# hammershock/3dgs-avatar-release

Measured on AMD Instinct MI355X. Metric: render fps (fwd+bwd) @200k Gaussians 1024x1024 SH3, higher is better.
Workload: dtype f32; 1 GPU; config3: 200k Gaussians, 1024x1024, SH deg 3, forward+backward; shs+scales+rotations inputs, L1 loss (L1 fused into the rasterizer: l1_target); tile_rect=1, l1=fused, long_lists=0, gaussians=200000, width=1024, height=1024, sh_degree=3, frames_per_rank=1857, total_frames=1857, ranks=1, backend=none, parallelism=frames sharded x1

## Files before the change

### 3dgs-avatar-release_amd/csrc/render_bwd.hip

```cpp
#include "common.h"
#include "blend.h"

__device__ __forceinline__ float ring_ror1(float v) {
    return __builtin_bit_cast(float, __builtin_amdgcn_update_dpp(0, __builtin_bit_cast(int, v), 0x121, 0xF, 0xF, true));
}
#define RING 16
#define RING_STRIDE 48

typedef float bwd_f4 __attribute__((ext_vector_type(4)));
template <bool SECOND>
__device__ __forceinline__ void split_accumulate(float (&x)[9], float (&y)[9], unsigned long long mask, float Gd, float dx,
                                                 float dy, float tdx, float tdy, float wgt, float gx, float gy,
                                                 float gz, unsigned long long m1, uint32_t lds_addr, bwd_f4& q0, bwd_f4& q1,
                                                 bwd_f4& q2, float& rot0, float& rot1) {
    unsigned long long save;
    asm volatile(
        "s_mov_b64 %[sv], exec\n\t"
        "s_mov_b64 exec, %[m]\n\t"
        "v_fmac_f32 %[x0], %[Gd], %[dx]\n\t"
        "v_fmac_f32 %[x1], %[Gd], %[dy]\n\t"
        "v_fmac_f32 %[x2], %[tdx], %[dx]\n\t"
        "v_fmac_f32 %[x3], %[tdx], %[dy]\n\t"
        "v_fmac_f32 %[x4], %[tdy], %[dy]\n\t"
        "v_add_f32 %[x5], %[x5], %[Gd]\n\t"
        "v_fmac_f32 %[x6], %[w], %[gx]\n\t"
        "v_fmac_f32 %[x7], %[w], %[gy]\n\t"
        "v_fmac_f32 %[x8], %[w], %[gz]\n\t"
        "s_mov_b64 exec, %[sv]"
        : [x0] "+v"(x[0]), [x1] "+v"(x[1]), [x2] "+v"(x[2]), [x3] "+v"(x[3]), [x4] "+v"(x[4]), [x5] "+v"(x[5]), [x6] "+v"(x[6]),
          [x7] "+v"(x[7]), [x8] "+v"(x[8]), [sv] "=&s"(save)
        : [m] "s"(mask), [Gd] "v"(Gd), [dx] "v"(dx), [dy] "v"(dy), [tdx] "v"(tdx), [tdy] "v"(tdy), [w] "v"(wgt), [gx] "v"(gx),
          [gy] "v"(gy), [gz] "v"(gz)
        : "scc");
#define GS_ACC_Y                                     \
        "s_andn2_b64 exec, %[sv], %[m]\n\t"          \
        "v_fmac_f32 %[y0], %[Gd], %[dx]\n\t"         \
        "v_fmac_f32 %[y1], %[Gd], %[dy]\n\t"         \
        "v_fmac_f32 %[y2], %[tdx], %[dx]\n\t"        \
        "v_fmac_f32 %[y3], %[tdx], %[dy]\n\t"        \
        "v_fmac_f32 %[y4], %[tdy], %[dy]\n\t"        \
        "v_add_f32 %[y5], %[y5], %[Gd]\n\t"          \
        "v_fmac_f32 %[y6], %[w], %[gx]\n\t"          \
        "v_fmac_f32 %[y7], %[w], %[gy]\n\t"          \
        "v_fmac_f32 %[y8], %[w], %[gz]\n\t"          \
        "s_mov_b64 exec, %[sv]\n\t"                  \
        "v_mov_b32_dpp %[r0], %[r0] row_ror:1 row_mask:0xf bank_mask:0xf bound_ctrl:1\n\t" \
        "v_mov_b32_dpp %[r1], %[r1] row_ror:1 row_mask:0xf bank_mask:0xf bound_ctrl:1\n\t" \
        "s_waitcnt lgkmcnt(0)"
#define GS_ACC_Y_OUT [y0] "+v"(y[0]), [y1] "+v"(y[1]), [y2] "+v"(y[2]), [y3] "+v"(y[3]), [y4] "+v"(y[4]), [y5] "+v"(y[5]), \
                     [y6] "+v"(y[6]), [y7] "+v"(y[7]), [y8] "+v"(y[8]), [q0] "+v"(q0), [q1] "+v"(q1), [r0] "+v"(rot0), [r1] "+v"(rot1), \
                     [sv] "=&s"(save)
#define GS_ACC_Y_IN [m] "s"(mask), [m1] "s"(m1), [a] "v"(lds_addr), [Gd] "v"(Gd), [dx] "v"(dx), [dy] "v"(dy), [tdx] "v"(tdx), \
                    [tdy] "v"(tdy), [w] "v"(wgt), [gx] "v"(gx), [gy] "v"(gy), [gz] "v"(gz)
    if constexpr (SECOND) {
        asm volatile(
            "s_mov_b64 %[sv], exec\n\t"
            "s_andn2_b64 exec, %[m1], %[m]\n\t"
            "ds_read_b128 %[q0], %[a]\n\t"
            "ds_read_b128 %[q1], %[a] offset:16\n\t"
            "ds_read_b128 %[q2], %[a] offset:32\n\t" GS_ACC_Y
            : GS_ACC_Y_OUT, [q2] "+v"(q2)
            : GS_ACC_Y_IN
            : "memory", "scc");
    } else {
        asm volatile(
            "s_mov_b64 %[sv], exec\n\t"
            "s_andn2_b64 exec, %[m1], %[m]\n\t"
            "ds_read_b128 %[q0], %[a]\n\t"
            "ds_read_b128 %[q1], %[a] offset:16\n\t"
            "ds_read_b32 %[q2], %[a] offset:32\n\t" GS_ACC_Y
            : GS_ACC_Y_OUT, [q2] "+v"(q2.x)
            : GS_ACC_Y_IN
            : "memory", "scc");
    }
#undef GS_ACC_Y
#undef GS_ACC_Y_OUT
#undef GS_ACC_Y_IN
}

struct EntryQ {
    bwd_f4 q0, q1, q2;
};
#define ENT_SLOTS 2

template <bool SECOND>
__device__ __forceinline__ void switch_entry(EntryQ& e, uint32_t lds_addr, unsigned long long m0, unsigned long long m1) {
    unsigned long long save;
    if constexpr (SECOND) {
        asm volatile(
            "s_mov_b64 %[sv], exec\n\t"
            "s_andn2_b64 exec, %[m1], %[m0]\n\t"
            "ds_read_b128 %[q0], %[a]\n\t"
            "ds_read_b128 %[q1], %[a] offset:16\n\t"
            "ds_read_b128 %[q2], %[a] offset:32\n\t"
            "s_mov_b64 exec, %[sv]\n\t"
            "s_waitcnt lgkmcnt(0)"
            : [q0] "+v"(e.q0), [q1] "+v"(e.q1), [q2] "+v"(e.q2), [sv] "=&s"(save)
            : [a] "v"(lds_addr), [m0] "s"(m0), [m1] "s"(m1)
            : "memory", "scc");
    } else {
        float b = e.q2.x;
        asm volatile(
            "s_mov_b64 %[sv], exec\n\t"
            "s_andn2_b64 exec, %[m1], %[m0]\n\t"
            "ds_read_b128 %[q0], %[a]\n\t"
            "ds_read_b128 %[q1], %[a] offset:16\n\t"
            "ds_read_b32 %[b], %[a] offset:32\n\t"
            "s_mov_b64 exec, %[sv]\n\t"
            "s_waitcnt lgkmcnt(0)"
            : [q0] "+v"(e.q0), [q1] "+v"(e.q1), [b] "+v"(b), [sv] "=&s"(save)
            : [a] "v"(lds_addr), [m0] "s"(m0), [m1] "s"(m1)
            : "memory", "scc");
        e.q2.x = b;
    }
}

#ifndef BWD_MIN_WAVES
#define BWD_MIN_WAVES 1
#endif
#ifndef BWD_MAX_WAVES
#define BWD_MAX_WAVES (BWD_MIN_WAVES > 6 ? BWD_MIN_WAVES : 6)
#endif
template <int MODE>
__attribute__((amdgpu_waves_per_eu(BWD_MIN_WAVES, BWD_MAX_WAVES)))
__global__ __launch_bounds__(64, BWD_MIN_WAVES) void render_bwd_kernel(const float4* __restrict__ rec,
                                                        const uint2* __restrict__ ranges,
                                                        const uint32_t* __restrict__ order, int W, int H, int gx,
                                                        int ntiles, int xmap,
                                                        const uint32_t* __restrict__ qlist,
                                                        const uint32_t* __restrict__ ncon_c,
                                                        const uint32_t* __restrict__ qcount,
                                                        const float* __restrict__ out_color,
                                                        const float* __restrict__ dL_dpix,
                                                        const float* __restrict__ dL_dopa,
                                                        const float* __restrict__ final_T, const float* __restrict__ bg,
                                                        float4* __restrict__ qrows, uint32_t* __restrict__ q8,
                                                        const float4* __restrict__ ckpt,
                                                        const uint32_t* __restrict__ ck_start, const int chunks,
                                                        const int blocks_per_chunk, const SecondImage second,
                                                        const L1Grad l1, const float l1_inv_n) {
    constexpr bool OPA = MODE == 1, SECOND = MODE == 2, SONES = MODE == 3;
    if constexpr (SECOND) { if (*second.all_ones != 0u) return; }
    if constexpr (SONES) { if (*second.all_ones == 0u) return; }
    constexpr int NP2 = SECOND ? 5 : 3;
    __shared__ float2 pix[NP2][4 * RING_STRIDE];
    __shared__ bwd_f4 ent[ENT_SLOTS][RING][3];
    int slot, q;
    const int chunk = chunks > 1 ? (int)blockIdx.x / blocks_per_chunk : 0;
    render_block_map((int)blockIdx.x - chunk * blocks_per_chunk, xmap, &slot, &q);
    if (slot >= ntiles) return;
    const int tile = (int)(order[slot] & 0x7FFFFFFFu);
    const int tx = tile % gx, ty = tile / gx;
    const int lane = threadIdx.x;
    const int j = lane & (RING - 1), ring = lane / RING;
    const int QX0 = tx * TILE + 8 * (q & 1), QY0 = ty * TILE + 8 * (q >> 1);
    const int pi = (RING - j) & (RING - 1), pl = ring * RING + pi;
    const int px = QX0 + (pl & 7), py = QY0 + (pl >> 3);
    const uint2 range = ranges[tile];
    const int n = (int)(range.y - range.x);
    const int m_all = (int)qcount[tile * 4 + q];
    const uint32_t ks = chunk > 0 ? ck_start[(size_t)(tile * 4 + q) * (size_t)chunks + chunk] : 0u;
    if (ks >= (uint32_t)m_all) return;
    const int k0 = (int)ks;
    const uint32_t ke = chunk + 1 < chunks ? ck_start[(size_t)(tile * 4 + q) * (size_t)chunks + chunk + 1] : 0xFFFFFFFFu;
    const int m = (int)min(ke, (uint32_t)m_all) - k0;
    if (m <= 0) return;
    const uint32_t qbase = 4u * range.x + (uint32_t)q * (uint32_t)n + (uint32_t)k0;
    const float4 zero4 = make_float4(0.f, 0.f, 0.f, 0.f);
    float gtot0, T0 = 1.0f;
    {
        float4 c0 = zero4, c1 = make_float4((float)px, (float)py, __uint_as_float((uint32_t)pi), 0.f);
        float3 h = make_float3(0.f, 0.f, 0.f);
        if (px < W && py < H) {
            const size_t HW = (size_t)H * W;
            const size_t pid = (size_t)py * W + px;
            float g0 = 0.f, g1 = 0.f, g2 = 0.f;
            if (dL_dpix) { g0 = dL_dpix[pid]; g1 = dL_dpix[HW + pid]; g2 = dL_dpix[2 * HW + pid]; }
            const float o0 = out_color[pid], o1 = out_color[HW + pid], o2 = out_color[2 * HW + pid];
            if (l1.target) {
                const float sc = (l1.grad ? l1.grad[0] : 1.0f) * l1_inv_n;
                const float d0 = o0 - l1.target[pid], d1 = o1 - l1.target[HW + pid], d2 = o2 - l1.target[2 * HW + pid];
                g0 += d0 > 0.f ? sc : (d0 < 0.f ? -sc : 0.f);
                g1 += d1 > 0.f ? sc : (d1 < 0.f ? -sc : 0.f);
                g2 += d2 > 0.f ? sc : (d2 < 0.f ? -sc : 0.f);
            }
            c0 = make_float4(g0, g1, g2, o0 * g0 + o1 * g1 + o2 * g2);
            const uint32_t nc = ncon_c[pid];
            c1.z = __uint_as_float((nc > (uint32_t)k0 ? nc - (uint32_t)k0 : 0u) + (uint32_t)pi);
            if (OPA) {
                const float Tf = final_T[pid];
                c0.w -= dL_dopa[pid] * (Tf * (1.0f - bg[0]));
            }
            if (SECOND || SONES) {
                h = make_float3(second.dL_dpix[pid], second.dL_dpix[HW + pid], second.dL_dpix[2 * HW + pid]);
                if (SECOND) c0.w += second.out_color[pid] * h.x + second.out_color[HW + pid] * h.y + second.out_color[2 * HW + pid] * h.z;
                else c0.w -= (1.0f - second.out_color[pid]) * h.x + (1.0f - second.out_color[HW + pid]) * h.y + (1.0f - second.out_color[2 * HW + pid]) * h.z;
            }
            if (chunk > 0) {
                const size_t ci = ((size_t)(tile * 4 + q) * (size_t)(chunks - 1) + (size_t)(chunk - 1)) * 64 + pl;
                const float4 ck = ckpt[ci];
                T0 = ck.x;
                c0.w -= ck.y * g0 + ck.z * g1 + ck.w * g2;
                if (SECOND) {
                    const float4 ck2 = second.ckpt[ci];
                    c0.w -= ck2.y * h.x + ck2.z * h.y + ck2.w * h.z;
                }
            }
        }
        const int slot = ring * RING_STRIDE + pi;
        pix[0][slot] = pix[0][slot + RING] = make_float2(c0.x, c0.y);
        pix[1][slot] = pix[1][slot + RING] = make_float2(c0.z, c1.x);
        pix[2][slot] = pix[2][slot + RING] = make_float2(c1.y, c1.z);
        if (SECOND) {
            pix[3][slot] = pix[3][slot + RING] = make_float2(h.x, h.y);
            pix[4][slot] = pix[4][slot + RING] = make_float2(h.z, 0.f);
        }
        gtot0 = c0.w;
    }

    float3 q2 = make_float3(0.f, 0.f, 0.f);
    auto stage = [&](const float4 p0, const float4 p1, const float4 p2, const int chunk, uint32_t& row) {
        const uint32_t off = __float_as_uint(p2.y), rmin = __float_as_uint(p2.z), rsz = __float_as_uint(p2.w);
        const uint32_t minx = rmin & 0xFFFFu, miny = rmin >> 16, w = rsz & 0xFFFFu;
        row = gradient_row(off, w, (uint32_t)tx - minx, (uint32_t)ty - miny, (uint32_t)q);
        if (ring == 0) {
            bwd_f4* e = ent[chunk & (ENT_SLOTS - 1)][j];
            e[0] = bwd_f4{p0.x, p0.y, (-0.5f * LOG2E_F) * p0.z, -LOG2E_F * p0.w};
            e[1] = bwd_f4{(-0.5f * LOG2E_F) * p1.x, p1.y, p1.z, p1.w};
            e[2] = bwd_f4{p2.x, q2.x, q2.y, q2.z};
        }
    };
    uint32_t id_ahead = 0;
    auto gather_id = [&](int k) { id_ahead = qlist[qbase + min(k, m - 1)]; };
    auto gather = [&](float4& p0, float4& p1, float4& p2) {
        const uint32_t id = id_ahead;
        p0 = rec[(size_t)id * 3];
        p1 = rec[(size_t)id * 3 + 1];
        p2 = rec[(size_t)id * 3 + 2];
        if (SECOND) q2 = make_float3(second.colors[(size_t)id * 3], second.colors[(size_t)id * 3 + 1], second.colors[(size_t)id * 3 + 2]);
    };

    float4 p0 = zero4, p1 = zero4, p2 = zero4;
    EntryQ cur;
    cur.q0 = cur.q1 = cur.q2 = bwd_f4{0.f, 0.f, 0.f, 0.f};
    uint32_t row_staged = 0;
    gather_id(j);
    gather(p0, p1, p2);
    gather_id(RING + j);
    stage(p0, p1, p2, 0, row_staged);
    gather(p0, p1, p2);
    gather_id(2 * RING + j);
    __syncthreads();
    const uint32_t ent_addr0 = (uint32_t)(uintptr_t)&ent[0][j][0], ent_addr1 = (uint32_t)(uintptr_t)&ent[1][j][0];

    float accA[9], accB[9];
#pragma unroll
    for (int c9 = 0; c9 < 9; c9++) accA[c9] = accB[c9] = 0.f;
    uint32_t rowA = 0, rowB = 0;
    uint32_t pidx = (uint32_t)(ring * RING_STRIDE + pi);
    float2 pc[NP2];
#pragma unroll
    for (int c6 = 0; c6 < NP2; c6++) pc[c6] = pix[c6][pidx];
    float T = T0, Rem = gtot0;

    auto fold_rings = [&](float (&a)[9], float (&f)[3]) {
        float t;
        asm volatile(
            "s_nop 1\n\t"
            "v_permlane16_swap_b32 %[a0], %[a1]\n\t"
            "v_permlane16_swap_b32 %[a2], %[a3]\n\t"
            "v_permlane16_swap_b32 %[a4], %[a5]\n\t"
            "v_permlane16_swap_b32 %[a6], %[a7]\n\t"
            "v_mov_b32 %[t], %[a8]\n\t"
            "v_add_f32 %[a0], %[a0], %[a1]\n\t"
            "v_add_f32 %[a2], %[a2], %[a3]\n\t"
            "v_add_f32 %[a4], %[a4], %[a5]\n\t"
            "v_add_f32 %[a6], %[a6], %[a7]\n\t"
            "v_permlane16_swap_b32 %[a8], %[t]\n\t"
            "v_permlane32_swap_b32 %[a0], %[a2]\n\t"
            "v_permlane32_swap_b32 %[a4], %[a6]\n\t"
            "v_add_f32 %[a8], %[a8], %[t]\n\t"
            "v_add_f32 %[a0], %[a0], %[a2]\n\t"
            "v_add_f32 %[a4], %[a4], %[a6]\n\t"
            "v_mov_b32 %[t], %[a8]\n\t"
            "s_nop 1\n\t"
            "v_permlane32_swap_b32 %[a8], %[t]\n\t"
            "v_add_f32 %[a8], %[a8], %[t]"
            : [a0] "+v"(a[0]), [a1] "+v"(a[1]), [a2] "+v"(a[2]), [a3] "+v"(a[3]), [a4] "+v"(a[4]), [a5] "+v"(a[5]),
              [a6] "+v"(a[6]), [a7] "+v"(a[7]), [a8] "+v"(a[8]), [t] "=&v"(t));
        f[0] = a[0];
        f[1] = a[4];
        f[2] = a[8];
    };
    float* const qrow_words = reinterpret_cast<float*>(qrows);
    auto write_row = [&](size_t row, const float (&f)[3]) {
        qrow_words[row * 8 + ring] = f[0];
        qrow_words[row * 8 + ring + 4] = f[1];
        if (ring == 0) q8[row] = __float_as_uint(f[2]);
    };

    const int total = m + RING - 1;
    auto run_round = [&](const int s0, float (&X)[9], uint32_t& rowX, float (&Y)[9]) {
        const uint32_t row_done = rowX;
        rowX = row_staged;
        const uint32_t ea = (s0 & RING) ? ent_addr1 : ent_addr0;
        switch_entry<SECOND>(cur, ea, 0ull, 0x0001000100010001ull);
        stage(p0, p1, p2, s0 / RING + 1, row_staged);
        gather(p0, p1, p2);
        gather_id(s0 + 3 * RING + j);
        if (s0 >= 2 * RING) {
            float f[3];
            fold_rings(X, f);
            write_row(row_done, f);
        }
        if (s0 > 0) pidx -= (uint32_t)RING;
#pragma unroll
        for (int c9 = 0; c9 < 9; c9++) X[c9] = 0.f;
        const int tend = min(RING, total - s0);
        unsigned long long mx = 0x0001000100010001ull;
        auto step = [&](const int t) {
            const uint32_t s = (uint32_t)(s0 + t);
            const float3 g = make_float3(pc[0].x, pc[0].y, pc[1].x);
            const float pxf = pc[1].y, pyf = pc[2].x;
            const uint32_t lim = __float_as_uint(pc[2].y);
            const float h0 = SECOND ? pc[3].x : 0.f, h1 = SECOND ? pc[3].y : 0.f, h2 = SECOND ? pc[NP2 - 1].x : 0.f;
            pidx += 1u;
#pragma unroll
            for (int c6 = 0; c6 < NP2; c6++) pc[c6] = pix[c6][pidx];
            const float dx = cur.q0.x - pxf, dy = cur.q0.y - pyf;
            const float power2 = __builtin_fmaf(cur.q0.z * dx, dx, __builtin_fmaf(cur.q0.w, dx, cur.q1.x * dy) * dy);
            const float G = __builtin_amdgcn_exp2f(power2);
            const float al = fminf(0.99f, cur.q1.y * G);
            const bool valid = (power2 <= 0.0f) && (s < lim) && (al >= (1.0f / 255.0f));
            const float alpha = valid ? al : 0.f;
            const float Gv = valid ? G : 0.f;
            const float wgt = alpha * T;
            float cg = cur.q1.z * g.x + cur.q1.w * g.y + cur.q2.x * g.z;
            if constexpr (SECOND) cg += cur.q2.y * h0 + cur.q2.z * h1 + cur.q2.w * h2;
            Rem = __builtin_fmaf(-cg, wgt, Rem);
            const float one_m = 1.f - alpha;
            const float dL_dalpha = T * cg - Rem * __builtin_amdgcn_rcpf(one_m);
            T *= one_m;
            const float Gd = Gv * dL_dalpha;
            const float tdx = Gd * dx, tdy = Gd * dy;
            const unsigned long long mx1 = (mx << 1) | 0x0001000100010001ull;
            split_accumulate<SECOND>(X, Y, mx, Gd, dx, dy, tdx, tdy, wgt, g.x, g.y, g.z, mx1, ea, cur.q0, cur.q1, cur.q2, T, Rem);
            mx = mx1;
        };
        int t = 0;
        for (; t + 1 < tend; t += 2) {
            step(t);
            step(t + 1);
        }
        if (t < tend) step(t);
    };
    for (int s0 = 0; s0 < total; s0 += 2 * RING) {
        run_round(s0, accA, rowA, accB);
        if (s0 + RING < total) run_round(s0 + RING, accB, rowB, accA);
    }
    {
        const int last_round = (total - 1) / RING;
        const bool odd = last_round & 1;
        const int k_new = RING * last_round + j, k_old = k_new - RING;
        float fA[3], fB[3];
        fold_rings(accA, fA);
        fold_rings(accB, fB);
        if (k_new <= m - 1) write_row(odd ? rowB : rowA, odd ? fB : fA);
        if (last_round >= 1 && k_old <= m - 1) write_row(odd ? rowA : rowB, odd ? fA : fB);
    }
}

int launch_render_backward(const float* rec, const uint32_t* ranges, const uint32_t* order, int W, int H,
                           const QuadLists& ql, const float* out_color, const float* dL_dpix, const float* dL_dopa,
                           const float* final_T, const float* bg, float* qrows, uint32_t* q8, const SecondImage* second,
                           L1Grad l1, hipStream_t s) {
    const int gx = (W + TILE - 1) / TILE, gy = (H + TILE - 1) / TILE;
    const int xmap = gs_tune_get(GS_TUNE_XCD_MAP);
    const int chunks = ql.ckpt ? ql.chunks : 1;
    const int bpc = render_grid_blocks(gx * gy, xmap);
    const dim3 grid((unsigned)bpc * (unsigned)chunks);
    const SecondImage none{nullptr, nullptr, nullptr, nullptr, nullptr};
    const float l1_inv_n = 1.0f / (3.0f * (float)W * (float)H);
#define GS_BWD_ARGS                                                                                                       \
    reinterpret_cast<const float4*>(rec), reinterpret_cast<const uint2*>(ranges), order, W, H, gx, gx * gy, xmap, ql.qlist, \
        ql.ncon_c, ql.qcount, out_color, dL_dpix, dL_dopa, final_T, bg, reinterpret_cast<float4*>(qrows), q8, ql.ckpt,    \
        ql.ck_start, chunks, bpc
    if (second) {
        hipLaunchKernelGGL(render_bwd_kernel<2>, grid, dim3(64), 0, s, GS_BWD_ARGS, *second, l1, l1_inv_n);
        hipLaunchKernelGGL(render_bwd_kernel<3>, grid, dim3(64), 0, s, GS_BWD_ARGS, *second, l1, l1_inv_n);
    } else if (dL_dopa)
        hipLaunchKernelGGL(render_bwd_kernel<1>, grid, dim3(64), 0, s, GS_BWD_ARGS, none, l1, l1_inv_n);
    else
        hipLaunchKernelGGL(render_bwd_kernel<0>, grid, dim3(64), 0, s, GS_BWD_ARGS, none, l1, l1_inv_n);
#undef GS_BWD_ARGS
    GS_LAUNCH_CHECK("render_backward", 0, s);
    return GS_OK;
}
```

### 3dgs-avatar-release_amd/csrc/render_fwd.hip

```cpp
#include "common.h"
#include "blend.h"
#include <type_traits>

struct FwdArgs {
    const float4* __restrict__ rec;
    const uint32_t* __restrict__ point_list;
    const uint2* __restrict__ ranges;
    const uint32_t* __restrict__ order;
    const float* __restrict__ bg;
    int W, H, gx, ntiles, xmap;
    float* __restrict__ out_color;
    float* __restrict__ final_T;
    uint32_t* __restrict__ n_contrib;
    uint32_t* __restrict__ qlist;
    uint32_t* __restrict__ ncon_c;
    uint32_t* __restrict__ qcount;
    float4* __restrict__ ckpt;
    uint32_t* __restrict__ ck_start;
    int chunks;
    const uint32_t* __restrict__ src_qcount;
    const uint32_t* __restrict__ src_n_contrib;
    const unsigned long long* __restrict__ not_ones;
    uint4* __restrict__ marks;
    size_t mark_quads;
    uint32_t* __restrict__ marks_flag;
    uint32_t* __restrict__ all_ones;
    const float* __restrict__ l1_target;
    float* __restrict__ l1_part;
};
__device__ __forceinline__ void forward_side_fill(const FwdArgs& A) {
    if (!A.marks) {
        if (A.marks_flag && blockIdx.x == 0 && threadIdx.x == 0) *A.marks_flag = 0u;
        return;
    }
    const uint4 ones = make_uint4(0xFFFFFFFFu, 0xFFFFFFFFu, 0xFFFFFFFFu, 0xFFFFFFFFu);
    for (size_t k = (size_t)blockIdx.x * blockDim.x + threadIdx.x; k < A.mark_quads; k += (size_t)gridDim.x * blockDim.x)
        store_stream(&A.marks[k], ones);
    if (blockIdx.x == 0 && threadIdx.x == 0) *A.marks_flag = MARKS_CLEAN;
}

__device__ __forceinline__ void wave_lds_sync() {
    __builtin_amdgcn_fence(__ATOMIC_ACQ_REL, "wavefront");
    __builtin_amdgcn_wave_barrier();
}

__device__ __forceinline__ void lds_barrier() {
    asm volatile("s_waitcnt lgkmcnt(0)\n\ts_barrier" ::: "memory");
}

template <bool FQ>
__device__ __forceinline__ void render_quadrant_1(const FwdArgs& A, const int tile, const int q, float4* __restrict__ srec) {
    const float4* __restrict__ rec = A.rec;
    const uint32_t* __restrict__ point_list = A.point_list;
    const float* __restrict__ bg = A.bg;
    const int W = A.W, H = A.H, gx = A.gx, chunks = A.chunks;
    float* __restrict__ out_color = A.out_color;
    float* __restrict__ final_T = A.final_T;
    uint32_t* __restrict__ n_contrib = A.n_contrib;
    uint32_t* __restrict__ qlist = A.qlist;
    uint32_t* __restrict__ ncon_c = A.ncon_c;
    uint32_t* __restrict__ qcount = A.qcount;
    float4* __restrict__ ckpt = A.ckpt;
    uint32_t* __restrict__ ck_start = A.ck_start;
    const int tx = tile % gx, ty = tile / gx;
    const int lane = threadIdx.x & 63;
    const int QX0 = tx * TILE + 8 * (q & 1), QY0 = ty * TILE + 8 * (q >> 1);
    const int px = QX0 + (lane & 7), py = QY0 + (lane >> 3);
    const float pxf = (float)px, pyf = (float)py;
    const bool inside = px < W && py < H;
    const uint2 range = A.ranges[tile];
    const int n_tile = (int)(range.y - range.x);
    const uint32_t qbase = 4u * range.x + (uint32_t)q * (uint32_t)n_tile;
    const int n = FQ ? (int)A.src_qcount[tile * 4 + q] : n_tile;
    const uint32_t* __restrict__ list = FQ ? qlist + qbase : point_list + range.x;
    const unsigned long long lt_mask = (lane == 0) ? 0ull : (~0ull >> (64 - lane));
    uint32_t vzero;
    asm volatile("v_mov_b32 %0, 0" : "=v"(vzero));

    float T = inside ? 1.0f : -1.0f, C0 = 0.f, C1 = 0.f, C2 = 0.f;
    float gt0 = 0.f, gt1 = 0.f, gt2 = 0.f;
    if (A.l1_target && inside) {
        const size_t HW = (size_t)H * W, pid = (size_t)py * W + px;
        gt0 = A.l1_target[pid]; gt1 = A.l1_target[HW + pid]; gt2 = A.l1_target[2 * HW + pid];
    }
    uint32_t last = 0, last_k = 0;
    uint32_t kcount = 0;
    int nck = 0;
    bool live = __ballot(T > 0.f) != 0ull;

    float4 p0 = make_float4(0, 0, 0, 0), p1 = p0, p2 = p0;
    uint32_t pid_g = 0, pid_n = 0;
    if (live && lane < n) {
        pid_g = list[lane];
        p0 = rec[(size_t)pid_g * 3];
        p1 = rec[(size_t)pid_g * 3 + 1];
        p2 = rec[(size_t)pid_g * 3 + 2];
    }
    if (live && 64 + lane < n) pid_n = list[64 + lane];
    for (int base = 0; base < n && live; base += 64) {
        asm volatile("" : "+v"(pid_n));
        Staged s;
        bool hit;
        if (FQ) {
            stage_entry_convert(p0, p1, p2, s);
            hit = base + lane < n;
        } else {
            hit = stage_entry_quad(p0, p1, p2, QX0, QY0, s) && (base + lane < n);
        }
        const unsigned long long bal = __ballot(hit);
        const int cnt = __popcll(bal);
        wave_lds_sync();
        if (hit) {
            const int slot = __popcll(bal & lt_mask);
            const uint32_t k = kcount + (uint32_t)slot;
            s.c.w = __uint_as_float((uint32_t)(base + lane + 1));
            srec[slot * 3] = s.a;
            srec[slot * 3 + 1] = s.b;
            srec[slot * 3 + 2] = s.c;
            if (!FQ) qlist[qbase + k] = pid_g;
        }
        wave_lds_sync();
        kcount += (uint32_t)cnt;
        if (base + 64 + lane < n) {
            pid_g = pid_n;
            p0 = rec[(size_t)pid_g * 3];
            p1 = rec[(size_t)pid_g * 3 + 1];
            p2 = rec[(size_t)pid_g * 3 + 2];
            if (base + 128 + lane < n) pid_n = list[base + 128 + lane];
        }
        const char* sp = reinterpret_cast<const char*>(srec) + vzero;
        const uint32_t kbase = kcount - (uint32_t)cnt;
        auto blend = [&](const float4 a, const float2 b, const float4 c, uint32_t& mark) {
            const float dx = a.x - pxf, dy = a.y - pyf;
            const float power2 = __builtin_fmaf(a.z * dx, dx, __builtin_fmaf(a.w, dx, b.x * dy) * dy);
            const float G = __builtin_amdgcn_exp2f(power2);
            const float al = fminf(0.99f, b.y * G);
            const bool valid = power2 <= 0.0f && al >= (1.0f / 255.0f);
            const float a2 = valid ? al : 0.f;
            const float test_T = T * (1.f - a2);
            const bool pass = test_T >= 0.0001f;
            const float wT = a2 * T;
            const float w = pass ? wT : 0.f;
            T = pass ? test_T : -fabsf(T);
            C0 += c.x * w;
            C1 += c.y * w;
            C2 += c.z * w;
            mark = (valid && pass) ? (uint32_t)(uintptr_t)sp : mark;
        };
        auto ld_a = [&](int o) { return *reinterpret_cast<const float4*>(sp + o); };
        auto ld_b = [&](int o) { return *reinterpret_cast<const float2*>(sp + o + 16); };
        auto ld_c = [&](int o) {
            const float4 c = *reinterpret_cast<const float4*>(sp + o + 32);
            asm volatile("" ::"v"(c.w));
            return c;
        };
        const uint32_t sp0 = (uint32_t)(uintptr_t)sp;
        uint32_t mark_e = mark_none_even(sp0), mark_o = mark_none_odd(sp0);
        auto run = [&](const int j0, const int j1) {
            float4 a0 = ld_a(0), c0 = ld_c(0);
            float2 b0 = ld_b(0);
            int j = j0;
            for (; j + 1 < j1; j += 2) {
                const float4 a1 = ld_a(48), c1 = ld_c(48);
                const float2 b1 = ld_b(48);
                blend(a0, b0, c0, mark_e);
                a0 = ld_a(96); c0 = ld_c(96); b0 = ld_b(96);
                sp += 96;
                blend(a1, b1, c1, mark_o);
            }
            if (j < j1) {
                blend(a0, b0, c0, mark_e);
                sp += 48;
            }
        };
        int jc = cnt;
        if (chunks > 1) {
            const uint32_t r = (BWD_CH - (kbase & (BWD_CH - 1u))) & (BWD_CH - 1u);
            if (r < (uint32_t)cnt && kbase + r > 0u && kbase + r < (uint32_t)chunks * BWD_CH) jc = (int)r;
        }
        run(0, jc);
        if (jc < cnt) {
            nck = (int)((kbase + (uint32_t)jc) / BWD_CH);
            ckpt[((size_t)(tile * 4 + q) * (size_t)(chunks - 1) + (size_t)(nck - 1)) * 64 + lane] = make_float4(fabsf(T), C0, C1, C2);
            if (lane == 0) ck_start[(size_t)(tile * 4 + q) * (size_t)chunks + nck] = kbase + (uint32_t)jc;
            run(jc, cnt);
        }
        const uint32_t jl = marks_last_entry(mark_e, mark_o, sp0);
        if (jl) {
            last_k = kbase + jl;
            last = __float_as_uint(srec[(jl - 1u) * 3 + 2].w);
        }
        live = __ballot(T > 0.f) != 0ull;
    }
    {
        const uint32_t nm = wave_max_u32(last_k);
        if (lane == 0) qcount[tile * 4 + q] = nm;
        if (chunks > 1 && lane > nck && lane < chunks) ck_start[(size_t)(tile * 4 + q) * (size_t)chunks + lane] = 0xFFFFFFFFu;
    }
    float l1 = 0.f;
    if (inside) {
        const size_t HW = (size_t)H * W;
        const size_t pid = (size_t)py * W + px;
        const float Tf = fabsf(T);
        final_T[pid] = Tf;
        n_contrib[pid] = FQ ? A.src_n_contrib[pid] : last;
        ncon_c[pid] = last_k;
        const float o0 = C0 + Tf * bg[0], o1 = C1 + Tf * bg[1], o2 = C2 + Tf * bg[2];
        out_color[pid] = o0;
        out_color[HW + pid] = o1;
        out_color[2 * HW + pid] = o2;
        l1 = (fabsf(o0 - gt0) + fabsf(o1 - gt1)) + fabsf(o2 - gt2);
    }
    if (A.l1_target) {
        l1 = wave_sum(l1);
        if (lane == 0) A.l1_part[tile * 4 + q] = l1;
    }
}

template <bool FQ>
__device__ __forceinline__ void render_fwd_body(const FwdArgs& A, float4* __restrict__ srec) {
    int slot, q;
    if (blockIdx.x == 0 && threadIdx.x == 0 && A.all_ones) *A.all_ones = (A.not_ones && *A.not_ones == 0ull) ? 1u : 0u;
    const int b = (int)blockIdx.x;
    const bool composite = !(FQ && A.not_ones && *A.not_ones == 0ull);
    render_block_map(b, A.xmap, &slot, &q);
    if (slot < A.ntiles && composite) {
        const uint32_t ov = A.order[slot];
        render_quadrant_1<FQ>(A, (int)(ov & 0x7FFFFFFFu), q, srec);
    }
    forward_side_fill(A);
}

template <bool FQ>
__global__ __launch_bounds__(64, 8) void render_fwd_kernel(const FwdArgs A) {
    __shared__ float4 srec[66 * 3];
    render_fwd_body<FQ>(A, srec);
}

template <int CTRL>
__device__ __forceinline__ float qperm(float v) {
    const int i = __builtin_bit_cast(int, v);
    return __builtin_bit_cast(float, __builtin_amdgcn_update_dpp(i, i, CTRL, 0xF, 0xF, false));
}
template <int CTRL>
__device__ __forceinline__ uint32_t qperm(uint32_t v) {
    return (uint32_t)__builtin_amdgcn_update_dpp((int)v, (int)v, CTRL, 0xF, 0xF, false);
}
__device__ __forceinline__ float mul_qprev(float t, float v) {
    const int i = __builtin_bit_cast(int, t);
    return __builtin_bit_cast(float, __builtin_amdgcn_update_dpp(i, i, 0x90, 0xF, 0xF, false)) * v;
}
#define QP_PREV 0x90
#define QP_PAIR 0x44
#define QP_X1 0xB1
#define QP_X2 0x4E
#define QP_LAST 0xFF
#define FWD4_BATCH 256

template <bool FQ>
__device__ __forceinline__ void render_quadrant_4(const FwdArgs& A, const int tile, const int q, float4* __restrict__ srec,
                                                  uint32_t* __restrict__ s_cnt, uint32_t* __restrict__ s_flag,
                                                  uint32_t* __restrict__ s_lastk) {
    const float4* __restrict__ rec = A.rec;
    const uint32_t* __restrict__ point_list = A.point_list;
    const uint2* __restrict__ ranges = A.ranges;
    const float* __restrict__ bg = A.bg;
    const int W = A.W, H = A.H, gx = A.gx, chunks = A.chunks;
    float* __restrict__ out_color = A.out_color;
    float* __restrict__ final_T = A.final_T;
    uint32_t* __restrict__ n_contrib = A.n_contrib;
    uint32_t* __restrict__ qlist = A.qlist;
    uint32_t* __restrict__ ncon_c = A.ncon_c;
    uint32_t* __restrict__ qcount = A.qcount;
    float4* __restrict__ ckpt = A.ckpt;
    uint32_t* __restrict__ ck_start = A.ck_start;
    const int tx = tile % gx, ty = tile / gx;
    const int tid = threadIdx.x, lane = tid & 63, wv = tid >> 6;
    const int p = lane >> 2, e = lane & 3;
    const bool e0 = e == 0;
    const uint32_t e0_mask = e0 ? 0xFFFFFFFFu : 0u;
    const int QX0 = tx * TILE + 8 * (q & 1), QY0 = ty * TILE + 8 * (q >> 1);
    const int px = QX0 + (p & 7), py = QY0 + 2 * wv + (p >> 3);
    const float pxf = (float)px, pyf = (float)py;
    const bool inside = px < W && py < H;
    const int pix_q = 16 * wv + p;
    const uint2 range = ranges[tile];
    const int n_tile = (int)(range.y - range.x);
    const uint32_t qbase = 4u * range.x + (uint32_t)q * (uint32_t)n_tile;
    const int n = FQ ? (int)A.src_qcount[tile * 4 + q] : n_tile;
    const uint32_t* __restrict__ list = FQ ? qlist + qbase : point_list + range.x;
    const size_t quad = (size_t)(tile * 4 + q);
    const unsigned long long lt_mask = (lane == 0) ? 0ull : (~0ull >> (64 - lane));

    float Tc = inside ? 1.0f : 0.0f, Tf = 1.0f, C0 = 0.f, C1 = 0.f, C2 = 0.f;
    float gt0 = 0.f, gt1 = 0.f, gt2 = 0.f;
    if (A.l1_target && inside && e0) {
        const size_t HW = (size_t)H * W, pid = (size_t)py * W + px;
        gt0 = A.l1_target[pid]; gt1 = A.l1_target[HW + pid]; gt2 = A.l1_target[2 * HW + pid];
    }
    uint32_t last = 0, last_k = 0;
    uint32_t kcount = 0;
    int nck = 0;
    bool live = QX0 < W && QY0 < H;

#ifdef FWD4_PROF
    unsigned long long pf_t0 = __builtin_readcyclecounter(), pf_stage = 0, pf_loop = 0, pf_tail = 0, pf_mark = 0;
    uint32_t pf_batches = 0, pf_steps = 0;
#define PF_MARK() (pf_mark = __builtin_readcyclecounter())
#define PF_ADD(x) do { const unsigned long long pf_n = __builtin_readcyclecounter(); x += pf_n - pf_mark; pf_mark = pf_n; } while (0)
#else
#define PF_MARK() ((void)0)
#define PF_ADD(x) ((void)0)
#endif
    float4 p0 = make_float4(0, 0, 0, 0), p1 = p0, p2 = p0;
    uint32_t pid_g = 0, pid_n = 0;
    if (live && tid < n) {
        pid_g = list[tid];
        p0 = rec[(size_t)pid_g * 3];
        p1 = rec[(size_t)pid_g * 3 + 1];
        p2 = rec[(size_t)pid_g * 3 + 2];
    }
    if (live && FWD4_BATCH + tid < n) pid_n = list[FWD4_BATCH + tid];
    for (int base = 0; base < n && live; base += FWD4_BATCH) {
        asm volatile("" : "+v"(pid_n));
        PF_MARK();
        Staged s;
        bool hit;
        if (FQ) {
            stage_entry_convert(p0, p1, p2, s);
            hit = base + tid < n;
        } else {
            hit = stage_entry_quad(p0, p1, p2, QX0, QY0, s) && (base + tid < n);
        }
        const unsigned long long bal = __ballot(hit);
        if (lane == 0) s_cnt[wv] = (uint32_t)__popcll(bal);
        lds_barrier();
        const uint32_t n0 = s_cnt[0], n1 = s_cnt[1], n2 = s_cnt[2], n3 = s_cnt[3];
        const int cnt = (int)(n0 + n1 + n2 + n3);
        const uint32_t woff = wv == 0 ? 0u : (wv == 1 ? n0 : (wv == 2 ? n0 + n1 : n0 + n1 + n2));
        const uint32_t lead = kcount & 3u;
        if (hit) {
            const uint32_t sl = woff + (uint32_t)__popcll(bal & lt_mask);
            s.c.w = __uint_as_float((uint32_t)(base + tid + 1));
            srec[(lead + sl) * 3] = s.a;
            srec[(lead + sl) * 3 + 1] = s.b;
            srec[(lead + sl) * 3 + 2] = s.c;
            if (!FQ) qlist[qbase + kcount + sl] = pid_g;
        }
        if (tid < 7) {
            const float4 z = make_float4(0.f, 0.f, 0.f, 0.f);
            const uint32_t zs = tid < 4 ? lead + (uint32_t)cnt + (uint32_t)tid : (uint32_t)tid - 4u;
            if (tid < 4 || zs < lead) {
                srec[zs * 3] = z;
                srec[zs * 3 + 1] = z;
                srec[zs * 3 + 2] = z;
            }
        }
        lds_barrier();
        const uint32_t kbase = kcount;
        kcount += (uint32_t)cnt;
        if (base + FWD4_BATCH + tid < n) {
            pid_g = pid_n;
            p0 = rec[(size_t)pid_g * 3];
            p1 = rec[(size_t)pid_g * 3 + 1];
            p2 = rec[(size_t)pid_g * 3 + 2];
            if (base + 2 * FWD4_BATCH + tid < n) pid_n = list[base + 2 * FWD4_BATCH + tid];
        }
        auto checkpoint = [&](const uint32_t k0) {
            float s0 = C0 + qperm<QP_X1>(C0), s1 = C1 + qperm<QP_X1>(C1), s2 = C2 + qperm<QP_X1>(C2);
            s0 += qperm<QP_X2>(s0);
            s1 += qperm<QP_X2>(s1);
            s2 += qperm<QP_X2>(s2);
            nck = (int)(k0 / BWD_CH);
            if (e0) ckpt[(quad * (size_t)(chunks - 1) + (size_t)(nck - 1)) * 64 + pix_q] = make_float4(Tc >= 0.0001f ? Tc : Tf, s0, s1, s2);
            if (tid == 0) ck_start[quad * (size_t)chunks + nck] = k0;
        };
        uint32_t ck_next = 0xFFFFFFFFu;
        if (chunks > 1) {
            const uint32_t k = (max(kbase, 1u) + BWD_CH - 1u) & ~(BWD_CH - 1u);
            if (k < (uint32_t)chunks * BWD_CH) ck_next = k;
        }
        auto ck_due = [&](const uint32_t k) {
            if (k != ck_next) return false;
            ck_next = (k + BWD_CH < (uint32_t)chunks * BWD_CH) ? k + BWD_CH : 0xFFFFFFFFu;
            return true;
        };
        PF_ADD(pf_stage);
#ifdef FWD4_PROF
        pf_batches++;
        pf_steps += (lead + (uint32_t)cnt + 3u) / 4u;
#endif
        const char* sp = reinterpret_cast<const char*>(srec) + e * 48;
        const uint32_t kstep0 = kbase - lead;
        const int nstaged = (int)lead + cnt;
        uint32_t idx1 = kstep0 + (uint32_t)e + 1u;
        auto step = [&](const float4 a, const float2 b, const float4 c) {
            const float dx = a.x - pxf, dy = a.y - pyf;
            const float power2 = __builtin_fmaf(a.z * dx, dx, __builtin_fmaf(a.w, dx, b.x * dy) * dy);
            const float G = __builtin_amdgcn_exp2f(power2);
            const float al = fminf(0.99f, b.y * G);
            const float a2 = (power2 <= 0.0f && al >= (1.0f / 255.0f)) ? al : 0.f;
            const float x = 1.f - a2;
            const float xs = __uint_as_float((__float_as_uint(qperm<QP_PREV>(x)) & ~e0_mask) | (0x3F800000u & e0_mask));
            float tb = Tc;
#pragma unroll
            for (int r = 0; r < 3; r++) tb = mul_qprev(tb, xs);
            const float ta = tb * x;
            const bool pass = ta >= 0.0001f;
            const float w = pass ? a2 * tb : 0.f;
            C0 += c.x * w;
            C1 += c.y * w;
            C2 += c.z * w;
            last_k = (w > 0.f) ? idx1 : last_k;
            idx1 += 4u;
            uint32_t cand = pass ? __float_as_uint(ta) : 0x7F800000u;
            cand = min(cand, qperm<QP_X1>(cand));
            cand = min(cand, qperm<QP_X2>(cand));
            Tf = cand != 0x7F800000u ? __uint_as_float(cand) : Tf;
            Tc = qperm<QP_LAST>(ta);
        };
        auto ld_a = [&](int o) { return *reinterpret_cast<const float4*>(sp + o); };
        auto ld_b = [&](int o) { return *reinterpret_cast<const float2*>(sp + o + 16); };
        auto ld_c = [&](int o) {
            const float4 c = *reinterpret_cast<const float4*>(sp + o + 32);
            asm volatile("" ::"v"(c.w));
            return c;
        };
        float4 a0 = ld_a(0), c0 = ld_c(0);
        float2 b0 = ld_b(0);
        int j = 0;
        for (; j + 4 < nstaged; j += 8) {
            if (ck_due(kstep0 + (uint32_t)j)) checkpoint(kstep0 + (uint32_t)j);
            const float4 a1 = ld_a(192), c1 = ld_c(192);
            const float2 b1 = ld_b(192);
            step(a0, b0, c0);
            if (ck_due(kstep0 + (uint32_t)j + 4u)) checkpoint(kstep0 + (uint32_t)j + 4u);
            a0 = ld_a(384); c0 = ld_c(384); b0 = ld_b(384);
            sp += 384;
            step(a1, b1, c1);
        }
        if (j < nstaged) {
            if (ck_due(kstep0 + (uint32_t)j)) checkpoint(kstep0 + (uint32_t)j);
            step(a0, b0, c0);
        }
        PF_ADD(pf_loop);
        {
            uint32_t lk = max(last_k, qperm<QP_X1>(last_k));
            lk = max(lk, qperm<QP_X2>(lk));
            last_k = lk;
            if (lk > kbase) last = __float_as_uint(srec[(lk - 1u - kstep0) * 3 + 2].w);
        }
        const bool alive = __ballot(Tc >= 0.0001f) != 0ull;
        if (lane == 0) s_flag[wv] = alive ? 1u : 0u;
        lds_barrier();
        live = (s_flag[0] | s_flag[1] | s_flag[2] | s_flag[3]) != 0u;
        PF_ADD(pf_tail);
    }
#ifdef FWD4_PROF
    if (tid == 0 && blockIdx.x < 8)
        printf("fwd4prof block %d tile %d q %d: list %d batches %u steps %u | cycles total %llu stage %llu loop %llu tail %llu\n", (int)blockIdx.x, tile, q, n,
               pf_batches, pf_steps, (unsigned long long)(__builtin_readcyclecounter() - pf_t0), pf_stage, pf_loop, pf_tail);
#endif
    {
        const uint32_t wm = wave_max_u32(last_k);
        if (lane == 0) s_lastk[wv] = wm;
        lds_barrier();
        if (tid == 0) qcount[quad] = max(max(s_lastk[0], s_lastk[1]), max(s_lastk[2], s_lastk[3]));
        if (chunks > 1 && tid > nck && tid < chunks) ck_start[quad * (size_t)chunks + tid] = 0xFFFFFFFFu;
    }
    float s0 = C0 + qperm<QP_X1>(C0), s1 = C1 + qperm<QP_X1>(C1), s2 = C2 + qperm<QP_X1>(C2);
// ... 83 lines not shown
```

Measured before the change: 1803 frames/s.

## Fully unroll backward ring round with constant LDS offsets and LDS-typed forward loads

The backward blend round is unrolled into 16 compile-time steps. Each step uses immediate ds_read offsets instead of choosing between two entry base addresses, and the per-step pixel index is computed directly rather than kept in a running counter. The final step of each round runs a new last_accumulate that prefetches the next buffer's entry, so the separate switch_entry call per round goes away and runs once before the loop. The non-SECOND staging path now writes only the one float it needs, and the forward kernel uses 32-bit LDS address-space pointers with the stride advance folded into an inline asm add. This cuts VALU/SALU address overhead in the hot loops, at the cost of larger code and more fragile hand-written asm ordering.

Measured after the change: 1821 frames/s (median of 6 runs). 1.0% higher.

```diff
diff --git a/3dgs-avatar-release_amd/csrc/render_bwd.hip b/3dgs-avatar-release_amd/csrc/render_bwd.hip
--- a/3dgs-avatar-release_amd/csrc/render_bwd.hip
+++ b/3dgs-avatar-release_amd/csrc/render_bwd.hip
@@ -8,7 +8,7 @@
 #define RING_STRIDE 48
 
 typedef float bwd_f4 __attribute__((ext_vector_type(4)));
-template <bool SECOND>
+template <bool SECOND, int OFF>
 __device__ __forceinline__ void split_accumulate(float (&x)[9], float (&y)[9], unsigned long long mask, float Gd, float dx,
                                                  float dy, float tdx, float tdy, float wgt, float gx, float gy,
                                                  float gz, unsigned long long m1, uint32_t lds_addr, bwd_f4& q0, bwd_f4& q1,
@@ -51,14 +51,15 @@
                      [y6] "+v"(y[6]), [y7] "+v"(y[7]), [y8] "+v"(y[8]), [q0] "+v"(q0), [q1] "+v"(q1), [r0] "+v"(rot0), [r1] "+v"(rot1), \
                      [sv] "=&s"(save)
 #define GS_ACC_Y_IN [m] "s"(mask), [m1] "s"(m1), [a] "v"(lds_addr), [Gd] "v"(Gd), [dx] "v"(dx), [dy] "v"(dy), [tdx] "v"(tdx), \
-                    [tdy] "v"(tdy), [w] "v"(wgt), [gx] "v"(gx), [gy] "v"(gy), [gz] "v"(gz)
+                    [tdy] "v"(tdy), [w] "v"(wgt), [gx] "v"(gx), [gy] "v"(gy), [gz] "v"(gz), [o0] "n"(OFF), [o1] "n"(OFF + 16), \
+                    [o2] "n"(OFF + 32)
     if constexpr (SECOND) {
         asm volatile(
             "s_mov_b64 %[sv], exec\n\t"
             "s_andn2_b64 exec, %[m1], %[m]\n\t"
-            "ds_read_b128 %[q0], %[a]\n\t"
-            "ds_read_b128 %[q1], %[a] offset:16\n\t"
-            "ds_read_b128 %[q2], %[a] offset:32\n\t" GS_ACC_Y
+            "ds_read_b128 %[q0], %[a] offset:%[o0]\n\t"
+            "ds_read_b128 %[q1], %[a] offset:%[o1]\n\t"
+            "ds_read_b128 %[q2], %[a] offset:%[o2]\n\t" GS_ACC_Y
             : GS_ACC_Y_OUT, [q2] "+v"(q2)
             : GS_ACC_Y_IN
             : "memory", "scc");
@@ -66,9 +67,9 @@
         asm volatile(
             "s_mov_b64 %[sv], exec\n\t"
             "s_andn2_b64 exec, %[m1], %[m]\n\t"
-            "ds_read_b128 %[q0], %[a]\n\t"
-            "ds_read_b128 %[q1], %[a] offset:16\n\t"
-            "ds_read_b32 %[q2], %[a] offset:32\n\t" GS_ACC_Y
+            "ds_read_b128 %[q0], %[a] offset:%[o0]\n\t"
+            "ds_read_b128 %[q1], %[a] offset:%[o1]\n\t"
+            "ds_read_b32 %[q2], %[a] offset:%[o2]\n\t" GS_ACC_Y
             : GS_ACC_Y_OUT, [q2] "+v"(q2.x)
             : GS_ACC_Y_IN
             : "memory", "scc");
@@ -78,8 +79,63 @@
 #undef GS_ACC_Y_IN
 }
 
+template <bool SECOND, int OFF>
+__device__ __forceinline__ void last_accumulate(float (&x)[9], float Gd, float dx, float dy, float tdx, float tdy, float wgt,
+                                                float gx, float gy, float gz, unsigned long long m0, uint32_t lds_addr,
+                                                bwd_f4& q0, bwd_f4& q1, bwd_f4& q2, float& rot0, float& rot1) {
+    unsigned long long save;
+#define GS_ACC_L                                     \
+        "s_mov_b64 exec, %[sv]\n\t"                  \
+        "v_fmac_f32 %[x0], %[Gd], %[dx]\n\t"         \
+        "v_fmac_f32 %[x1], %[Gd], %[dy]\n\t"         \
+        "v_fmac_f32 %[x2], %[tdx], %[dx]\n\t"        \
+        "v_fmac_f32 %[x3], %[tdx], %[dy]\n\t"        \
+        "v_fmac_f32 %[x4], %[tdy], %[dy]\n\t"        \
+        "v_add_f32 %[x5], %[x5], %[Gd]\n\t"          \
+        "v_fmac_f32 %[x6], %[w], %[gx]\n\t"          \
+        "v_fmac_f32 %[x7], %[w], %[gy]\n\t"          \
+        "v_fmac_f32 %[x8], %[w], %[gz]\n\t"          \
+        "v_mov_b32_dpp %[r0], %[r0] row_ror:1 row_mask:0xf bank_mask:0xf bound_ctrl:1\n\t" \
+        "v_mov_b32_dpp %[r1], %[r1] row_ror:1 row_mask:0xf bank_mask:0xf bound_ctrl:1\n\t"
+#define GS_ACC_L_OUT [x0] "+v"(x[0]), [x1] "+v"(x[1]), [x2] "+v"(x[2]), [x3] "+v"(x[3]), [x4] "+v"(x[4]), [x5] "+v"(x[5]), \
+                     [x6] "+v"(x[6]), [x7] "+v"(x[7]), [x8] "+v"(x[8]), [q0] "+v"(q0), [q1] "+v"(q1), [r0] "+v"(rot0), [r1] "+v"(rot1), \
+                     [sv] "=&s"(save)
+#define GS_ACC_L_IN [m0] "s"(m0), [a] "v"(lds_addr), [Gd] "v"(Gd), [dx] "v"(dx), [dy] "v"(dy), [tdx] "v"(tdx), [tdy] "v"(tdy), \
+                    [w] "v"(wgt), [gx] "v"(gx), [gy] "v"(gy), [gz] "v"(gz), [o0] "n"(OFF), [o1] "n"(OFF + 16), [o2] "n"(OFF + 32)
+    if constexpr (SECOND) {
+        asm volatile(
+            "s_mov_b64 %[sv], exec\n\t"
+            "s_mov_b64 exec, %[m0]\n\t"
+            "ds_read_b128 %[q0], %[a] offset:%[o0]\n\t"
+            "ds_read_b128 %[q1], %[a] offset:%[o1]\n\t"
+            "ds_read_b128 %[q2], %[a] offset:%[o2]\n\t" GS_ACC_L
+            "s_waitcnt lgkmcnt(0)"
+            : GS_ACC_L_OUT, [q2] "+v"(q2)
+            : GS_ACC_L_IN
+            : "memory");
+    } else {
+        asm volatile(
+            "s_mov_b64 %[sv], exec\n\t"
+            "s_mov_b64 exec, %[m0]\n\t"
+            "ds_read_b128 %[q0], %[a] offset:%[o0]\n\t"
+            "ds_read_b128 %[q1], %[a] offset:%[o1]\n\t"
+            "ds_read_b32 %[q2], %[a] offset:%[o2]\n\t" GS_ACC_L
+            "s_waitcnt lgkmcnt(0)"
+            : GS_ACC_L_OUT, [q2] "+v"(q2.x)
+            : GS_ACC_L_IN
+            : "memory");
+    }
+#undef GS_ACC_L
+#undef GS_ACC_L_OUT
+#undef GS_ACC_L_IN
+}
+
 struct EntryQ {
     bwd_f4 q0, q1, q2;
+};
+template <int V>
+struct bwd_const {
+    static constexpr int value = V;
 };
 #define ENT_SLOTS 2
 
@@ -227,7 +283,8 @@
             bwd_f4* e = ent[chunk & (ENT_SLOTS - 1)][j];
             e[0] = bwd_f4{p0.x, p0.y, (-0.5f * LOG2E_F) * p0.z, -LOG2E_F * p0.w};
             e[1] = bwd_f4{(-0.5f * LOG2E_F) * p1.x, p1.y, p1.z, p1.w};
-            e[2] = bwd_f4{p2.x, q2.x, q2.y, q2.z};
+            if constexpr (SECOND) e[2] = bwd_f4{p2.x, q2.x, q2.y, q2.z};
+            else *reinterpret_cast<float*>(e + 2) = p2.x;
         }
     };
     uint32_t id_ahead = 0;
@@ -251,16 +308,15 @@
     gather(p0, p1, p2);
     gather_id(2 * RING + j);
     __syncthreads();
-    const uint32_t ent_addr0 = (uint32_t)(uintptr_t)&ent[0][j][0], ent_addr1 = (uint32_t)(uintptr_t)&ent[1][j][0];
+    const uint32_t ent_addr0 = (uint32_t)(uintptr_t)&ent[0][j][0];
+    constexpr int ENT_SLOT_BYTES = RING * 3 * (int)sizeof(bwd_f4);
 
     float accA[9], accB[9];
 #pragma unroll
     for (int c9 = 0; c9 < 9; c9++) accA[c9] = accB[c9] = 0.f;
     uint32_t rowA = 0, rowB = 0;
-    uint32_t pidx = (uint32_t)(ring * RING_STRIDE + pi);
+    const uint32_t pbase = (uint32_t)(ring * RING_STRIDE + pi);
     float2 pc[NP2];
-#pragma unroll
-    for (int c6 = 0; c6 < NP2; c6++) pc[c6] = pix[c6][pidx];
     float T = T0, Rem = gtot0;
 
     auto fold_rings = [&](float (&a)[9], float (&f)[3]) {
@@ -300,11 +356,12 @@
     };
 
     const int total = m + RING - 1;
-    auto run_round = [&](const int s0, float (&X)[9], uint32_t& rowX, float (&Y)[9]) {
+    constexpr unsigned long long POS0 = 0x0001000100010001ull;
+    auto round_start = [&](const int s0, float (&X)[9], uint32_t& rowX) {
+#pragma unroll
+        for (int c6 = 0; c6 < NP2; c6++) pc[c6] = pix[c6][pbase];
         const uint32_t row_done = rowX;
         rowX = row_staged;
-        const uint32_t ea = (s0 & RING) ? ent_addr1 : ent_addr0;
-        switch_entry<SECOND>(cur, ea, 0ull, 0x0001000100010001ull);
         stage(p0, p1, p2, s0 / RING + 1, row_staged);
         gather(p0, p1, p2);
         gather_id(s0 + 3 * RING + j);
@@ -313,50 +370,73 @@
             fold_rings(X, f);
             write_row(row_done, f);
         }
-        if (s0 > 0) pidx -= (uint32_t)RING;
 #pragma unroll
         for (int c9 = 0; c9 < 9; c9++) X[c9] = 0.f;
-        const int tend = min(RING, total - s0);
-        unsigned long long mx = 0x0001000100010001ull;
-        auto step = [&](const int t) {
-            const uint32_t s = (uint32_t)(s0 + t);
-            const float3 g = make_float3(pc[0].x, pc[0].y, pc[1].x);
-            const float pxf = pc[1].y, pyf = pc[2].x;
-            const uint32_t lim = __float_as_uint(pc[2].y);
-            const float h0 = SECOND ? pc[3].x : 0.f, h1 = SECOND ? pc[3].y : 0.f, h2 = SECOND ? pc[NP2 - 1].x : 0.f;
-            pidx += 1u;
+    };
+    auto step = [&](const uint32_t s, const uint32_t pnext, const unsigned long long mx, float (&X)[9], float (&Y)[9], auto off,
+                    auto last) {
+        constexpr int OFF = decltype(off)::value;
+        const float3 g = make_float3(pc[0].x, pc[0].y, pc[1].x);
+        const float pxf = pc[1].y, pyf = pc[2].x;
+        const uint32_t lim = __float_as_uint(pc[2].y);
+        const float h0 = SECOND ? pc[NP2 - 2].x : 0.f, h1 = SECOND ? pc[NP2 - 2].y : 0.f, h2 = SECOND ? pc[NP2 - 1].x : 0.f;
+        if constexpr (!decltype(last)::value) {
 #pragma unroll
-            for (int c6 = 0; c6 < NP2; c6++) pc[c6] = pix[c6][pidx];
-            const float dx = cur.q0.x - pxf, dy = cur.q0.y - pyf;
-            const float power2 = __builtin_fmaf(cur.q0.z * dx, dx, __builtin_fmaf(cur.q0.w, dx, cur.q1.x * dy) * dy);
-            const float G = __builtin_amdgcn_exp2f(power2);
-            const float al = fminf(0.99f, cur.q1.y * G);
-            const bool valid = (power2 <= 0.0f) && (s < lim) && (al >= (1.0f / 255.0f));
-            const float alpha = valid ? al : 0.f;
-            const float Gv = valid ? G : 0.f;
-            const float wgt = alpha * T;
-            float cg = cur.q1.z * g.x + cur.q1.w * g.y + cur.q2.x * g.z;
-            if constexpr (SECOND) cg += cur.q2.y * h0 + cur.q2.z * h1 + cur.q2.w * h2;
-            Rem = __builtin_fmaf(-cg, wgt, Rem);
-            const float one_m = 1.f - alpha;
-            const float dL_dalpha = T * cg - Rem * __builtin_amdgcn_rcpf(one_m);
-            T *= one_m;
-            const float Gd = Gv * dL_dalpha;
-            const float tdx = Gd * dx, tdy = Gd * dy;
-            const unsigned long long mx1 = (mx << 1) | 0x0001000100010001ull;
-            split_accumulate<SECOND>(X, Y, mx, Gd, dx, dy, tdx, tdy, wgt, g.x, g.y, g.z, mx1, ea, cur.q0, cur.q1, cur.q2, T, Rem);
-            mx = mx1;
-        };
-        int t = 0;
-        for (; t + 1 < tend; t += 2) {
-            step(t);
-            step(t + 1);
+            for (int c6 = 0; c6 < NP2; c6++) pc[c6] = pix[c6][pnext];
         }
-        if (t < tend) step(t);
-    };
-    for (int s0 = 0; s0 < total; s0 += 2 * RING) {
-        run_round(s0, accA, rowA, accB);
-        if (s0 + RING < total) run_round(s0 + RING, accB, rowB, accA);
+        const float dx = cur.q0.x - pxf, dy = cur.q0.y - pyf;
+        const float power2 = __builtin_fmaf(cur.q0.z * dx, dx, __builtin_fmaf(cur.q0.w, dx, cur.q1.x * dy) * dy);
+        const float G = __builtin_amdgcn_exp2f(power2);
+        const float al = fminf(0.99f, cur.q1.y * G);
+        const bool valid = (power2 <= 0.0f) && (s < lim) && (al >= (1.0f / 255.0f));
+        const float alpha = valid ? al : 0.f;
+        const float Gv = valid ? G : 0.f;
+        const float wgt = alpha * T;
+        float cg = cur.q1.z * g.x + cur.q1.w * g.y + cur.q2.x * g.z;
+        if constexpr (SECOND) cg += cur.q2.y * h0 + cur.q2.z * h1 + cur.q2.w * h2;
+        Rem = __builtin_fmaf(-cg, wgt, Rem);
+        const float one_m = 1.f - alpha;
+        const float dL_dalpha = T * cg - Rem * __builtin_amdgcn_rcpf(one_m);
+        T *= one_m;
+        const float Gd = Gv * dL_dalpha;
+        const float tdx = Gd * dx, tdy = Gd * dy;
+        if constexpr (decltype(last)::value)
+            last_accumulate<SECOND, ENT_SLOT_BYTES - OFF>(X, Gd, dx, dy, tdx, tdy, wgt, g.x, g.y, g.z, POS0, ent_addr0, cur.q0,
+                                                          cur.q1, cur.q2, T, Rem);
+        else
+            split_accumulate<SECOND, OFF>(X, Y, mx, Gd, dx, dy, tdx, tdy, wgt, g.x, g.y, g.z, (mx << 1) | POS0, ent_addr0,
+                                          cur.q0, cur.q1, cur.q2, T, Rem);
+    };
+    auto run_round = [&](const int s0, float (&X)[9], uint32_t& rowX, float (&Y)[9], auto off) {
+        round_start(s0, X, rowX);
+        const int left = total - s0;
+#define GS_STEP(t)                                                                                                         \
+    step((uint32_t)(s0 + (t)), pbase + (uint32_t)((t) + 1), ((1ull << ((t) + 1)) - 1ull) * POS0, X, Y, off,                \
+         bwd_const<(t) == RING - 1>{});                                                                                    \
+    if (left <= (t) + 1) return true
+        GS_STEP(0);
+        GS_STEP(1);
+        GS_STEP(2);
+        GS_STEP(3);
+        GS_STEP(4);
+        GS_STEP(5);
+        GS_STEP(6);
+        GS_STEP(7);
+        GS_STEP(8);
+        GS_STEP(9);
+        GS_STEP(10);
+        GS_STEP(11);
+        GS_STEP(12);
+        GS_STEP(13);
+        GS_STEP(14);
+        GS_STEP(15);
+        return false;
+#undef GS_STEP
+    };
+    switch_entry<SECOND>(cur, ent_addr0, 0ull, POS0);
+    for (int s0 = 0;; s0 += 2 * RING) {
+        if (run_round(s0, accA, rowA, accB, bwd_const<0>{})) break;
+        if (run_round(s0 + RING, accB, rowB, accA, bwd_const<ENT_SLOT_BYTES>{})) break;
     }
     {
         const int last_round = (total - 1) / RING;
diff --git a/3dgs-avatar-release_amd/csrc/render_fwd.hip b/3dgs-avatar-release_amd/csrc/render_fwd.hip
--- a/3dgs-avatar-release_amd/csrc/render_fwd.hip
+++ b/3dgs-avatar-release_amd/csrc/render_fwd.hip
@@ -128,7 +128,7 @@
             p2 = rec[(size_t)pid_g * 3 + 2];
             if (base + 128 + lane < n) pid_n = list[base + 128 + lane];
         }
-        const char* sp = reinterpret_cast<const char*>(srec) + vzero;
+        uint32_t sp = (uint32_t)(uintptr_t)srec + vzero;
         const uint32_t kbase = kcount - (uint32_t)cnt;
         auto blend = [&](const float4 a, const float2 b, const float4 c, uint32_t& mark) {
             const float dx = a.x - pxf, dy = a.y - pyf;
@@ -145,16 +145,30 @@
             C0 += c.x * w;
             C1 += c.y * w;
             C2 += c.z * w;
-            mark = (valid && pass) ? (uint32_t)(uintptr_t)sp : mark;
-        };
-        auto ld_a = [&](int o) { return *reinterpret_cast<const float4*>(sp + o); };
-        auto ld_b = [&](int o) { return *reinterpret_cast<const float2*>(sp + o + 16); };
+            mark = (valid && pass) ? sp : mark;
+        };
+        typedef float lds_v4 __attribute__((ext_vector_type(4)));
+        typedef float lds_v2 __attribute__((ext_vector_type(2)));
+        auto ld4 = [&](int o) {
+            const lds_v4 v = *(const __attribute__((address_space(3))) lds_v4*)(sp + o);
+            return make_float4(v.x, v.y, v.z, v.w);
+        };
+        auto ld_a = [&](int o) { return ld4(o); };
+        auto ld_b = [&](int o) {
+            const lds_v2 v = *(const __attribute__((address_space(3))) lds_v2*)(sp + o + 16);
+            return make_float2(v.x, v.y);
+        };
         auto ld_c = [&](int o) {
-            const float4 c = *reinterpret_cast<const float4*>(sp + o + 32);
+            const float4 c = ld4(o + 32);
             asm volatile("" ::"v"(c.w));
             return c;
         };
-        const uint32_t sp0 = (uint32_t)(uintptr_t)sp;
+        auto ld_c_advance = [&](int o, uint32_t& mark) {
+            const float4 c = ld4(o + 32);
+            asm volatile("v_add_u32 %0, 0x60, %0" : "+v"(sp), "+v"(mark) : "v"(c.w));
+            return c;
+        };
+        const uint32_t sp0 = sp;
         uint32_t mark_e = mark_none_even(sp0), mark_o = mark_none_odd(sp0);
         auto run = [&](const int j0, const int j1) {
             float4 a0 = ld_a(0), c0 = ld_c(0);
@@ -164,8 +178,7 @@
                 const float4 a1 = ld_a(48), c1 = ld_c(48);
                 const float2 b1 = ld_b(48);
                 blend(a0, b0, c0, mark_e);
-                a0 = ld_a(96); c0 = ld_c(96); b0 = ld_b(96);
-                sp += 96;
+                a0 = ld_a(96); b0 = ld_b(96); c0 = ld_c_advance(96, mark_e);
                 blend(a1, b1, c1, mark_o);
             }
             if (j < j1) {
```
